# croci/bluest

Hardware: AMD Instinct MI355X
Metric: Phi-assemblies/s (higher is better)
Workload: dtype f64; 1 GPU; n=20 models, groups up to size 5 (K_tot=21699), n_out=8, Wishart covariances; one step = V and grad V of one allocation for all outputs; n_models=20, k_max=5, K_tot=21699, n_out=8, batch=1, parallelism=single GPU, evaluation=stored group inverses, launch=hipGraph replay of 20-step graphs (20 of 20 steps), rest eager

## Files before the change

bluest_amd/csrc/plan.hip:

```cpp

#include "common.hpp"

static int g_debug_timing = getenv("BLUEST_DEBUG_TIMING") ? 1 : 0;
struct PhaseTimer {
    std::chrono::steady_clock::time_point t0 = std::chrono::steady_clock::now();
    const char *what;
    explicit PhaseTimer(const char *w) : what(w) {}
    void lap(const char *phase)
    {
        if (!g_debug_timing) return;
        const auto t1 = std::chrono::steady_clock::now();
        fprintf(stderr, "[bluest timing] %s: %s %.3f ms\n", what, phase, std::chrono::duration<double, std::milli>(t1 - t0).count());
        t0 = t1;
    }
};


#include "plan.hpp"
#include "spg_state.hpp"

template <typename COLT> __device__ __forceinline__ int4 load_cols4(const COLT *p);
template <> __device__ __forceinline__ int4 load_cols4<int32_t>(const int32_t *p) { return *reinterpret_cast<const int4 *>(p); }
template <> __device__ __forceinline__ int4 load_cols4<uint16_t>(const uint16_t *p)
{
// ... 139 lines not shown
                                                           double *__restrict__ v, int32_t *__restrict__ status,
                                                           const int32_t *__restrict__ gate, double *__restrict__ spg_state, int last_slot, int32_t *__restrict__ spg_enable,
                                                           unsigned int *__restrict__ ticket)
{
    __shared__ SolveLds<NT> lds;
    __shared__ double spg_ls[SPG_STATE_DOUBLES];
    __shared__ int s_closed;
    kernarg_now(N, n_out, rows, nsym, reg.Cd, reg.Co, reg.rank_ab, partial, n_chunks, gate, spg_state);
    const int o = blockIdx.x, c = blockIdx.y, tid = threadIdx.x;
    if (gate_closed(gate, &s_closed)) {
        if (spg_state && tid < WAVE && spg_closed_last(ticket + 16, gridDim.x * gridDim.y, tid))
            spg_decide_wave(spg_state, var, status, n_out, last_slot, spg_enable, spg_ls, tid);
        return;
    }
    SpgPrefetch pf;
    if (spg_state && tid < WAVE) spg_prefetch_state(spg_state, tid, pf);
    if (N < NT) { clear_pads(lds, N, tid, fold_threads(NT)); __syncthreads(); }
    fold_rows(lds, N, rows, o, nsym, partial + (int64_t)c * n_chunks, tid, fold_threads(NT), reg);
    __syncthreads();
    if (tid >= WAVE) return;
    const int lane = tid;
    if (spg_state) spg_prefetch_parts(pf, lane);
    const int64_t e = (int64_t)c * n_out + o;
    if (want_v & 2) {
        if (lane == 0) { var[e] = lds.at(0, 0); status[e] = 0; }
        return;
    }
    const double am = (lane < N) ? lds.amax[lane] : 0.0;
    const bool big = __ballot(am >= 0.05) != 0ull;
    const int reps = (want_v & 4) ? 2 : 1;
    double V_mine = 0.0;
    int32_t st_mine = 0;
    for (int rep = 0; rep < reps; rep++)
        solve_wave<NT>(lds, N, delta, am > 1.0e-6, am > 0.0, big, (want_v & 1) != 0, &V_mine, v + e * N, &st_mine, lane);
    if (lane == 0) { var[e] = V_mine; status[e] = st_mine; }
    if (spg_state) {
        int last = 0;
        if (n_out == 1) {
            spg_decide_wave(spg_state, var, status, n_out, last_slot, spg_enable, spg_ls, lane, pf, true, V_mine, st_mine);
            return;
        }
        if (lane == 0) {
            asm volatile("s_waitcnt vmcnt(0)" ::: "memory");
            __builtin_amdgcn_fence(__ATOMIC_RELEASE, "agent");
            asm volatile("s_waitcnt vmcnt(0)" ::: "memory");
            const unsigned int t = __hip_atomic_fetch_add(ticket, 1u, __ATOMIC_RELAXED, __HIP_MEMORY_SCOPE_AGENT);
            last = (t == (unsigned int)(n_out - 1)) ? 1 : 0;
            if (last) __hip_atomic_store(ticket, 0u, __ATOMIC_RELAXED, __HIP_MEMORY_SCOPE_AGENT);
        }
        last = __builtin_amdgcn_readfirstlane(last);
        if (last) {
            __builtin_amdgcn_fence(__ATOMIC_ACQUIRE, "agent");
            spg_decide_wave(spg_state, var, status, n_out, last_slot, spg_enable, spg_ls, lane, pf);
        }
    }
}

template <int NT>
__global__ __launch_bounds__(fold_threads(NT)) void k_fold_to_record(int N, int n_out, const RowDesc *__restrict__ rows, int nsym, FoldReg reg,
                                                        const double2 *__restrict__ partial, int64_t n_chunks,
                                                        double *__restrict__ rec)
{
    __shared__ SolveLds<NT> lds;
    kernarg_now(N, n_out, rows, nsym, reg.Cd, reg.Co, reg.rank_ab, partial, n_chunks, rec);
    const int o = blockIdx.x, c = blockIdx.y, tid = threadIdx.x;
    fold_rows(lds, N, rows, o, nsym, partial + (int64_t)c * n_chunks, tid, fold_threads(NT), reg);
    __syncthreads();
    const int reclen = N * N + 2 * N + 1;
    double *r = rec + ((int64_t)c * n_out + o) * reclen;
    for (int t = tid; t < N * N; t += fold_threads(NT)) r[t] = lds.at(t / N, t % N);
    if (tid >= WAVE) return;
    const double am = (tid < N) ? lds.amax[tid] : 0.0;
    if (tid < N) { r[N * N + tid] = (am > 1.0e-6) ? 1.0 : 0.0; r[N * N + N + tid] = (am > 0.0) ? 1.0 : 0.0; }
    const double big = wave_max(am);
    if (tid == 0) r[N * N + 2 * N] = (big >= 0.05) ? 1.0 : 0.0;
}

template <int NT>
__global__ __launch_bounds__(64) void k_solve_from_record(int N, int n_out, const double *__restrict__ rec,
                                                          double delta, int want_v, double *__restrict__ var,
                                                          double *__restrict__ v, int32_t *__restrict__ status)
{
    __shared__ SolveLds<NT> lds;
    const int o = blockIdx.x, c = blockIdx.y, lane = threadIdx.x;
    const int reclen = N * N + 2 * N + 1;
    const double *r = rec + ((int64_t)c * n_out + o) * reclen;
    clear_pads(lds, N, lane, WAVE);
    __syncthreads();
    for (int t = lane; t < N * N; t += WAVE) lds.at(t / N, t % N) = r[t];
    __syncthreads();
    const bool s1 = lane < N && r[N * N + lane] > 0.0;
    const bool s2 = lane < N && r[N * N + N + lane] > 0.0;
    const bool big = r[N * N + 2 * N] > 0.0;
    const int64_t e = (int64_t)c * n_out + o;
    solve_wave<NT>(lds, N, delta, s1, s2, big, (want_v & 1) != 0, var + e, v + e * N, status + e, lane);
}

__device__ __forceinline__ void jacobi_pinv_lds(double *A, double *Q, int N, int LD, int lane)
{
    for (int sweep = 0; sweep < 60; sweep++) {
        int rotated = 0;
        for (int p = 0; p < N - 1; p++)
            for (int q = p + 1; q < N; q++) {
                const double apq = A[p * LD + q], app = A[p * LD + p], aqq = A[q * LD + q];
                if (!(fabs(apq) > 1.0e-18 * sqrt(fabs(app * aqq)))) continue;
                rotated = 1;
                const double theta = (aqq - app) / (2.0 * apq);
                const double t = (theta >= 0 ? 1.0 : -1.0) / (fabs(theta) + sqrt(theta * theta + 1.0));
                const double c = 1.0 / sqrt(t * t + 1.0), sn = t * c;
                if (lane < N) {
                    const double arp = A[lane * LD + p], arq = A[lane * LD + q];
                    A[lane * LD + p] = c * arp - sn * arq;
                    A[lane * LD + q] = sn * arp + c * arq;
                    const double vrp = Q[lane * LD + p], vrq = Q[lane * LD + q];
                    Q[lane * LD + p] = c * vrp - sn * vrq;
                    Q[lane * LD + q] = sn * vrp + c * vrq;
                }
                wave_lds_sync();
                if (lane < N) {
                    const double apr = A[p * LD + lane], aqr = A[q * LD + lane];
                    A[p * LD + lane] = c * apr - sn * aqr;
                    A[q * LD + lane] = sn * apr + c * aqr;
                }
                wave_lds_sync();
            }
        if (!rotated) break;
    }
}
// ... 55 lines not shown
            }
            wave_lds_sync();
        }
    }
    if (lane < N) v[e * N + lane] = vmine;
    if (lane == 0) { var[e] = V; status[e] = st; }
}

template <int KU>
__global__ __launch_bounds__(256) void k_grad_tiles(const TileDesc *__restrict__ tiles, int64_t n_tiles,
                                                    const double *__restrict__ tvals, const double *__restrict__ v,
                                                    const int32_t *__restrict__ status, int N, int n_out, int n_cand,
                                                    double *__restrict__ grad, int64_t grad_stride,
                                                    const int32_t *__restrict__ gate)
{
    if (gate && *gate == 0) return;
    const int64_t t = (int64_t)blockIdx.x * 4 + (threadIdx.x >> 6);
    const int lane = threadIdx.x & 63;
    if (t >= n_tiles) return;
    const TileDesc td = tiles[t];
#define GT(KK) case KK: if (KK <= KU) { grad_tile<(KK <= KU ? KK : 1)>(td, tvals, v, status, N, n_out, n_cand, grad, grad_stride, lane); break; }
    switch (td.k) {
        GT(1) GT(2) GT(3) GT(4) GT(5) GT(6) GT(7) GT(8) GT(9) GT(10) GT(11) GT(12)
        default: grad_tile_generic(td, tvals, v, status, N, n_out, n_cand, grad, grad_stride, lane);
    }
#undef GT
}

__host__ __device__ constexpr int fused_tpb(int NT, int KU) { return (NT <= 26 && KU <= 8) ? 15 : 7; }
using SolveGradKuSet = InstSet<5, 6, 8, 12>;
using GradTilesKuSet = InstSet<5, 8, 12>;
using PhiObSet = InstSet<2, 4, 8>;
template <class F> static void solve_grad_ku_dispatch(int kmax, F &&launch) { SolveGradKuSet::dispatch(kmax, launch); }
constexpr uint32_t SG_HAS_REC = 1u, SG_HAS_GATE = 2u, SG_HAS_SPG = 4u;
template <int NT, int KU>
__global__ __launch_bounds__(64 * (fused_tpb(NT, KU) + 1)) void k_solve_grad(const double2 *__restrict__ partial, const uint16_t *__restrict__ rank_ab,
                                                    const RowDesc *__restrict__ rows, const TileDesc *__restrict__ tiles,
                                                    uint32_t n_nsym, int Cd, int Co, int bpo, uint32_t flags,
                                                    int n_out_arg, int tpb_arg, int tile_nt, const double *__restrict__ rec_arg, double delta,
                                                    const double *__restrict__ tvals,
                                                    double *__restrict__ var, double *__restrict__ v_ws,
                                                    int32_t *__restrict__ status, double *__restrict__ grad,
                                                    const int32_t *__restrict__ gate, double *__restrict__ spg_state_arg, int last_slot,
                                                    int32_t *__restrict__ spg_enable, unsigned int *__restrict__ ticket, const MaTail ma)
{
    constexpr int FUSED_TPB = fused_tpb(NT, KU);
    constexpr int NTHREADS = 64 * (FUSED_TPB + 1);
    constexpr int PU = tile_pairs(KU);
    __shared__ SolveLds<NT> lds;
    __shared__ double spg_ls[SPG_STATE_DOUBLES];
    const int N = (int)(n_nsym & 0xffu), nsym = (int)(n_nsym >> 8);
    const FoldReg reg{Cd, Co, rank_ab};
    const int tid = threadIdx.x, lane = tid & 63;
    const int wave = __builtin_amdgcn_readfirstlane(tid >> 6);
    int o, first, wg;
    if (bpo > 0) { o = blockIdx.y; first = blockIdx.x == 0; wg = o * bpo + blockIdx.x; }
    else { wg = blockIdx.x; const TileDesc td0 = tile_desc_uniform(tiles, (int64_t)wg * tpb_arg); o = td0.out; first = (td0.n_valid >> 30) & 1; }
    __shared__ int s_closed;
    double *spg_state = nullptr;
    if (flags & (SG_HAS_GATE | SG_HAS_SPG)) {
        if (flags & SG_HAS_SPG) spg_state = spg_state_arg;
        if ((flags & SG_HAS_GATE) && gate_closed(gate, &s_closed)) {
            if (spg_state && first && wave == 0 && spg_closed_last(ticket + 16, (unsigned int)n_out_arg, lane))
                spg_decide_wave(spg_state, var, status, n_out_arg, last_slot, spg_enable, spg_ls, lane);
            return;
        }
    }
    SpgPrefetch pf;
    if (spg_state && first && wave == 0) spg_prefetch_state(spg_state, lane, pf);
    if (N < NT) { clear_pads(lds, N, tid, NTHREADS); __syncthreads(); }
    const double *rec_o = (flags & SG_HAS_REC) ? rec_arg + (int64_t)o * (N * N + 2 * N + 1) : nullptr;
    if (rec_o) {
        for (int t = tid; t < N * N; t += NTHREADS) lds.at(t / N, t % N) = rec_o[t];
    } else {
        fold_rows<NT>(lds, N, rows, o, nsym, partial, tid, NTHREADS, reg,
                      [&]() { kernarg_now(n_out_arg, tpb_arg, delta, var, v_ws, status); });
    }
    const int n_out = uniform_value_here(n_out_arg), tpb = uniform_value_here(tpb_arg);
    const int64_t t0 = (int64_t)wg * tpb;
    TileDesc td;
    td.k = 1; td.n_valid = 0; td.val_off = td.grad_off = 0; td.out = (int16_t)o;
    if (wave > 0 && wave <= tpb) td = tile_desc_uniform(tiles, t0 + wave - 1);
    __syncthreads();
    const int k = td.k;
    double2 pr[PU];
    double V_pub = 0.0;
    int32_t st_pub = 0;
    if (wave == 0) {
        if (spg_state && first) spg_prefetch_parts(pf, lane);
        bool s1, s2, big;
        if (rec_o) {
            s1 = lane < N && rec_o[N * N + lane] > 0.0;
            s2 = lane < N && rec_o[N * N + N + lane] > 0.0;
            big = rec_o[N * N + 2 * N] > 0.0;
        } else {
            const double am = (lane < N) ? lds.amax[lane] : 0.0;
            s1 = am > 1.0e-6;
            s2 = am > 0.0;
            big = __ballot(am >= 0.05) != 0ull;
        }
        double V = 0.0;
        int32_t st = 0;
        solve_wave<NT>(lds, N, delta, s1, s2, big, true, &V, lds.vout, &st, lane);
        if (lane == 0) { lds.status = st; if (ma.x) lds.scratch[0] = V; }
        V_pub = V; st_pub = st;
        if (first) {
            if (lane == 0) { var[o] = V; status[o] = st; }
            if (lane < N) v_ws[(int64_t)o * N + lane] = lds.vout[lane];
        }
    } else if (k <= KU) {
        if (tile_nt) tile_load<PU, true>(pr, tvals + td.val_off, lane, tile_pairs(k));
        else tile_load(pr, tvals + td.val_off, lane, tile_pairs(k));
    }
    __syncthreads();
    if (wave == 0) {
        if (spg_state && first) {
            int last = 0;
            if (n_out == 1) {
                spg_decide_wave(spg_state, var, status, n_out, last_slot, spg_enable, spg_ls, lane, pf, true, V_pub, st_pub);
                return;
            }
            if (lane == 0) {
                asm volatile("s_waitcnt vmcnt(0)" ::: "memory");
                __builtin_amdgcn_fence(__ATOMIC_RELEASE, "agent");
                asm volatile("s_waitcnt vmcnt(0)" ::: "memory");
                const unsigned int t = __hip_atomic_fetch_add(ticket, 1u, __ATOMIC_RELAXED, __HIP_MEMORY_SCOPE_AGENT);
                last = (t == (unsigned int)(n_out - 1)) ? 1 : 0;
                if (last) __hip_atomic_store(ticket, 0u, __ATOMIC_RELAXED, __HIP_MEMORY_SCOPE_AGENT);
            }
            last = __builtin_amdgcn_readfirstlane(last);
            if (last) {
                __builtin_amdgcn_fence(__ATOMIC_ACQUIRE, "agent");
                spg_decide_wave(spg_state, var, status, n_out, last_slot, spg_enable, spg_ls, lane, pf);
            }
        }
        return;
    }
    const bool valid = lane < (td.n_valid & 0xffff);
    const bool inf = lds.status == BLUEST_EVAL_INF;
    double *gout = grad + td.grad_off + lane;
    const bool MA_ON = ma.x != nullptr;
#define GT(KK) case KK: if (KK <= KU) { const double q = tile_form<(KK <= KU ? KK : 1)>(pr, lds.vout);                                          \
        if (valid && !MA_ON) *gout = inf ? INFINITY : -q;                                                                                        \
        else if (valid && lds.status == BLUEST_EVAL_OK) { const int64_t i = td.grad_off + lane; const double so = ma.s[0], cci = ma.cc[i];       \
            const double xn = ma.x[i] * cci * ((1.0 / so) * q) / (lds.scratch[0] / so); ma.x[i] = xn; ma.m[i] = cci * xn; } break; }
    switch (k) {
        GT(1) GT(2) GT(3) GT(4) GT(5) GT(6) GT(7) GT(8) GT(9) GT(10) GT(11) GT(12)
        default: {
            const double *vl = lds.vout - (int64_t)td.out * N;
            const int32_t *sl = &lds.status - td.out;
            grad_tile_generic(td, tvals, vl, sl, N, n_out, 1, grad, 0, lane);
        }
    }
#undef GT
}

__global__ void k_combine_grad(const double *__restrict__ grad, int64_t grad_stride, const int64_t *__restrict__ goff,
                               const int32_t *__restrict__ invmap, int64_t L, int n_out,
                               const double *__restrict__ coef, const double *__restrict__ scale, int n_cand,
                               double *__restrict__ out, int64_t out_stride, const int32_t *__restrict__ gate)
{
    if (gate && *gate == 0) return;
    const int64_t j = (int64_t)blockIdx.x * blockDim.x + threadIdx.x;
    const int c = blockIdx.y;
    if (j >= L || c >= n_cand) return;
    double s = 0.0;
    for (int o = 0; o < n_out; o++) {
        const int32_t li = invmap[(int64_t)o * L + j];
        if (li >= 0) s = fma(coef[(int64_t)c * n_out + o], grad[(int64_t)c * grad_stride + goff[o] + li], s);
    }
    out[(int64_t)c * out_stride + j] = scale ? scale[j] * s : s;
}

// ... 690 lines not shown
extern "C" int bluest_plan_finalize(bluest_plan_t plan, int max_candidates)
{
    if (!plan) return fail(BLUEST_ERR_ARG, "plan is NULL");
    if (plan->finalized) return fail(BLUEST_ERR_STATE, "plan already finalized");
    if (plan->outs.empty()) return fail(BLUEST_ERR_STATE, "plan has no outputs");
    if (max_candidates <= 0 || max_candidates > 65535) return fail(BLUEST_ERR_ARG, "max_candidates=%d out of range", max_candidates);
    const int N = plan->N, n_out = (int)plan->outs.size();
    PhaseTimer timer("plan_finalize");

    plan->nsym = N * (N + 1) / 2;
    if (N > 64 || plan->nsym > 2080) return fail(BLUEST_ERR_ARG, "N=%d: the fused kernel's argument word holds N <= 64, nsym <= 2080", N);
    plan->max_cand = max_candidates;
    plan->shared = true;
    for (int o = 1; o < n_out; o++) {
        const OutputDesc &x = plan->outs[0], &y = plan->outs[o];
        if (x.K != y.K || x.sizes != y.sizes || x.groups != y.groups || x.mapping != y.mapping) { plan->shared = false; break; }
    }
    PlanLayout lay(n_out, plan->nsym, plan->shared ? 1 : n_out);
    int rc;
    if ((rc = layout_tiles(plan, lay))) return rc;
    plan->identity = plan->shared && plan->outs[0].L_o == plan->L;
    for (int64_t li = 0; plan->identity && li < plan->L; li++) plan->identity = plan->outs[0].mapping[li] == li;
    if ((rc = layout_phi(plan, lay, timer))) return rc;
    layout_fold_reg(plan, lay);
    timer.lap("CSR slots + columns");
    layout_invmap(plan, lay);
    plan->cols16 = plan->L <= 65536 && getenv("BLUEST_COLS32") == nullptr;
    plan->phi_ob_forced = 0;
    if (const char *e = getenv("BLUEST_PHI_OB")) { const int v = atoi(e); if (v == 2 || v == 4 || v == 8) plan->phi_ob_forced = v; }
    plan->phi_bytes = plan->n_chunks * lay.CH * 8 + (plan->shared ? plan->n_chunks / n_out : plan->n_chunks) * lay.CH * (plan->cols16 ? 2 : 4) + plan->n_chunks * 16;
    plan->grad_bytes = (int64_t)lay.n_tvals * 8 + plan->grad_len * 8;
    const char *nt_env = getenv("BLUEST_TILE_NT");
    plan->tile_nt = nt_env ? atoi(nt_env) != 0 : true;
    timer.lap("tile descriptors + inverse maps");
    if ((rc = arena_upload(plan, lay))) return rc;
    timer.lap("device arena + small uploads");
    if ((rc = scatter_values(plan, lay))) return rc;
    plan->finalized = true;
    if ((rc = mf_finalize(plan))) return rc;

    timer.lap("device scatter of the values");
    return BLUEST_OK;
}

int plan_ready(bluest_plan_t plan, int n_cand)
{
    if (!plan) return fail(BLUEST_ERR_ARG, "plan is NULL");
    if (!plan->finalized) return fail(BLUEST_ERR_STATE, "plan not finalized");
    if (n_cand <= 0 || n_cand > plan->max_cand) return fail(BLUEST_ERR_ARG, "n_cand=%d outside 1..%d", n_cand, plan->max_cand);
    return BLUEST_OK;
}

extern "C" int bluest_plan_output_layout(bluest_plan_t plan, int output, int *K, int64_t *sizes, int64_t *mapping)
{
    if (!plan || !K) return fail(BLUEST_ERR_ARG, "null pointer");
    if (output < 0 || output >= (int)plan->outs.size()) return fail(BLUEST_ERR_ARG, "output %d out of range", output);
    const OutputDesc &od = plan->outs[output];
    *K = od.K;
    if (sizes) std::copy(od.sizes.begin(), od.sizes.end(), sizes);
    if (mapping) std::copy(od.mapping.begin(), od.mapping.end(), mapping);
    return BLUEST_OK;
}

extern "C" int bluest_plan_restrict(bluest_plan_t parent, const int64_t *keep, int64_t n_keep, int max_candidates, bluest_plan_t *restricted)
{
    if (!parent || !keep || !restricted) return fail(BLUEST_ERR_ARG, "null pointer");
// ... 91 lines not shown
    return BLUEST_OK;
}

extern "C" int bluest_plan_traffic(bluest_plan_t plan, int64_t *phi_bytes, int64_t *grad_bytes)
{
    if (!plan) return fail(BLUEST_ERR_ARG, "plan is NULL");
    if (!plan->finalized) return fail(BLUEST_ERR_STATE, "plan not finalized");
    if (phi_bytes) *phi_bytes = plan->phi_bytes;
    if (grad_bytes) *grad_bytes = plan->grad_bytes;
    return BLUEST_OK;
}

extern "C" int bluest_plan_phi_len(bluest_plan_t plan, int64_t *len)
{
    if (!plan || !len) return fail(BLUEST_ERR_ARG, "null pointer");
    *len = (int64_t)plan->outs.size() * (plan->N * plan->N + 2 * plan->N + 1);
    return BLUEST_OK;
}

static void launch_grad(bluest_plan_t plan, const double *v_dev, const int32_t *status_dev, int n_cand, double *grad_dev,
                        int64_t grad_stride, hipStream_t st)
{
    GradTilesKuSet::dispatch(plan->kmax, [&](auto ku) {
        hipLaunchKernelGGL((k_grad_tiles<decltype(ku)::value>), dim3((unsigned)((plan->n_tiles + 3) / 4)), dim3(256), 0, st, plan->d_tiles,
                           plan->n_tiles, plan->d_tvals, v_dev, status_dev, plan->N, (int)plan->outs.size(), n_cand, grad_dev, grad_stride, plan->gate);
    });
}

static void launch_solve_from_record(bluest_plan_t plan, const double *rec, int n_cand, double delta, int want_v, double *var_dev,
                                     double *v_dev, int32_t *status_dev, hipStream_t st)
{
    const int n_out = (int)plan->outs.size();
    nt_dispatch(plan->N, [&](auto nt) {
        hipLaunchKernelGGL((k_solve_from_record<decltype(nt)::value>), dim3(n_out, n_cand), dim3(64), 0, st, plan->N, n_out, rec, delta, want_v,
                           var_dev, v_dev, status_dev);
    });
}

static void launch_solve_grad(bluest_plan_t plan, const double *rec, double delta, double *var_dev, int32_t *status_dev, double *grad_dev,
                              double *dec_state, int dec_last, int32_t *dec_enable, MaTail ma, hipStream_t st)
{
    const int n_out = (int)plan->outs.size();
    const dim3 grid = plan->fused_bpo > 0 ? dim3((unsigned)plan->fused_bpo, (unsigned)n_out) : dim3((unsigned)(plan->n_tiles / plan->fused_tpb));
    const uint32_t flags = (rec ? SG_HAS_REC : 0u) | (plan->gate ? SG_HAS_GATE : 0u) | (dec_state ? SG_HAS_SPG : 0u);
    nt_dispatch(plan->N, [&](auto nt) { solve_grad_ku_dispatch(plan->kmax, [&](auto ku) {
        constexpr int NT = decltype(nt)::value, KU = decltype(ku)::value;
        hipLaunchKernelGGL((k_solve_grad<NT, KU>), grid, dim3(64 * (fused_tpb(NT, KU) + 1)), 0, st, plan->d_partial, plan->fold_reg.rank_ab, plan->d_rows,
                           plan->d_tiles, (uint32_t)plan->N | (uint32_t)plan->nsym << 8, plan->fold_reg.Cd, plan->fold_reg.Co, plan->fused_bpo, flags,
                           n_out, plan->fused_tpb, (int)plan->tile_nt, rec, delta, plan->d_tvals, var_dev, plan->d_v, status_dev, grad_dev,
                           plan->gate, dec_state, dec_last, dec_enable, plan->d_ticket, ma);
    }); });
}

static const int64_t PHI_MIN_WAVES = 2304;
static int phi_ob(const bluest_plan_s *p, int n_cand)
{
    (void)n_cand;
    const int n_out = (int)p->outs.size();
    if (!p->shared || n_out < 2) return 0;
    if (p->phi_ob_forced) return p->phi_ob_forced;
    const int64_t ncpo = p->n_chunks / n_out;
    for (int i = PhiObSet::count - 1; i > 0; i--) {
        const int ob = PhiObSet::values[i];
        if (ob <= n_out && ncpo * ((n_out + ob - 1) / ob) >= PHI_MIN_WAVES) return ob;
    }
    return PhiObSet::values[0];
}

static void launch_chunks(bluest_plan_t p, const double *m, int n_cand, int64_t m_stride, hipStream_t st)
{
    const int n_out = (int)p->outs.size();
    const uint32_t flags = p->gate ? PHI_HAS_GATE : 0u;
    if (const int ob = phi_ob(p, n_cand)) {
        const int64_t ncpo = p->n_chunks / n_out;
        PhiObSet::dispatch(ob, [&](auto obc) {
            constexpr int OB = decltype(obc)::value;
#define LCS2(COLT) hipLaunchKernelGGL((k_phi_chunks_shared<OB, 1, COLT>), dim3((unsigned)ncpo, (n_out + OB - 1) / OB), dim3(64), 0, st, \
// ... 112 lines not shown
{
    if (!state_dev || !enable_dev || !status_dev || !grad_dev) return fail(BLUEST_ERR_ARG, "null pointer");
    if (plan && (int)plan->outs.size() > SPG_MAX_OUT) return fail(BLUEST_ERR_ARG, "more than %d outputs", SPG_MAX_OUT);
    return plan_eval(plan, m_dev, 1, 0, delta, var_dev, grad_dev, plan ? plan->grad_len : 0, status_dev, stream, state_dev, last_slot, enable_dev);
}

static int plan_eval(bluest_plan_t plan, const double *m_dev, int n_cand, int64_t m_stride, double delta,
                     double *var_dev, double *grad_dev, int64_t grad_stride, int32_t *status_dev, void *stream,
                     double *dec_state, int dec_last, int32_t *dec_enable, MaTail ma)
{
    int rc = plan_ready(plan, n_cand); if (rc) return rc;
    if (!m_dev || !var_dev) return fail(BLUEST_ERR_ARG, "null pointer");
    if (n_cand > 1 && m_stride < plan->L) return fail(BLUEST_ERR_ARG, "m_stride < L_global");
    if (grad_dev && n_cand > 1 && grad_stride < plan->grad_len) return fail(BLUEST_ERR_ARG, "grad_stride < grad_len");
    hipStream_t st = (hipStream_t)stream;
    const int n_out = (int)plan->outs.size();
    int32_t *status = status_dev ? status_dev : plan->d_status;
    if (plan->matfree && n_cand == 1 && !dec_state && !plan->gate) {
        const double *rec = nullptr;
        if ((rc = mf_phi_record(plan, m_dev, nullptr, &rec, st))) return rc;
        if (grad_dev) return mf_solve_grad(plan, rec, delta, var_dev, status, grad_dev, st, ma);
        launch_solve_from_record(plan, rec, 1, delta, plan->always_v ? 1 : 0, var_dev, plan->d_v, status, st);
        HIP_TRY(hipGetLastError());
        return BLUEST_OK;
    }
    launch_chunks(plan, m_dev, n_cand, m_stride, st);
    if (plan->mf_gradient && grad_dev && n_cand == 1 && !dec_state && !plan->gate)
        return mf_solve_grad(plan, nullptr, delta, var_dev, status, grad_dev, st, ma);
    if (grad_dev && n_cand == 1) {
        launch_solve_grad(plan, nullptr, delta, var_dev, status, grad_dev, dec_state, dec_last, dec_enable, ma, st);
        HIP_TRY(hipGetLastError());
        return BLUEST_OK;
    }
    const int want = (grad_dev || plan->always_v) ? 1 : 0;
    nt_dispatch(plan->N, [&](auto nt) {
        hipLaunchKernelGGL((k_solve_from_chunks<decltype(nt)::value>), dim3(n_out, n_cand), dim3(fold_threads(nt)), 0, st, plan->N, n_out, plan->d_rows,
                           plan->nsym, plan->fold_reg, plan->d_partial, plan->partial_stride, delta, want, var_dev, plan->d_v, status, plan->gate,
                           dec_state, dec_last, dec_enable, plan->d_ticket);
    });
    if (grad_dev)
        launch_grad(plan, plan->d_v, status, n_cand, grad_dev, grad_stride, st);
    HIP_TRY(hipGetLastError());
    return BLUEST_OK;
}

extern "C" int bluest_plan_is_identity(bluest_plan_t plan, int *yes)
{
    if (!plan || !yes) return fail(BLUEST_ERR_ARG, "null pointer");
    if (!plan->finalized) return fail(BLUEST_ERR_STATE, "plan not finalized");
    *yes = plan->identity ? 1 : 0;
    return BLUEST_OK;
}

static int eval_ma_kmax(const bluest_plan_s *plan)
{
    if (plan->outs.size() != 1 || !plan->identity || plan->gate) return 0;
    return plan->matfree ? 8 : 12;
}

extern "C" int bluest_plan_eval_ma_kmax(bluest_plan_t plan, int *kmax)
{
    if (!plan || !kmax) return fail(BLUEST_ERR_ARG, "null pointer");
    if (!plan->finalized) return fail(BLUEST_ERR_STATE, "plan not finalized");
    *kmax = eval_ma_kmax(plan);
    return BLUEST_OK;
}

extern "C" int bluest_plan_kmax(bluest_plan_t plan, int *kmax)
{
    if (!plan || !kmax) return fail(BLUEST_ERR_ARG, "null pointer");
    if (!plan->finalized) return fail(BLUEST_ERR_STATE, "plan not finalized");
    *kmax = plan->kmax;
    return BLUEST_OK;
}

extern "C" int bluest_plan_launch_config(bluest_plan_t plan, int n_cand, int32_t *cfg)
{
    if (!plan || !cfg) return fail(BLUEST_ERR_ARG, "null pointer");
    if (!plan->finalized) return fail(BLUEST_ERR_STATE, "plan not finalized");
    if (n_cand <= 0 || n_cand > plan->max_cand) return fail(BLUEST_ERR_ARG, "n_cand=%d outside 1..%d", n_cand, plan->max_cand);
    std::fill(cfg, cfg + BLUEST_LC_COUNT, 0);
    const bool one = n_cand == 1 && !plan->gate;
    cfg[BLUEST_LC_PATH] = (one && plan->matfree) ? 2 : (one && plan->mf_gradient) ? 3 : (n_cand == 1) ? 1 : 0;
    cfg[BLUEST_LC_PHI_OB] = phi_ob(plan, n_cand);
    cfg[BLUEST_LC_COLS16] = plan->cols16 ? 1 : 0;
    nt_dispatch(plan->N, [&](auto nt) {
        cfg[BLUEST_LC_NT] = decltype(nt)::value;
        cfg[BLUEST_LC_FOLD_THREADS] = fold_threads(decltype(nt)::value);
        solve_grad_ku_dispatch(plan->kmax, [&](auto ku) {
            cfg[BLUEST_LC_SOLVE_GRAD_KU] = decltype(ku)::value;
            cfg[BLUEST_LC_FUSED_TPB] = fused_tpb(decltype(nt)::value, decltype(ku)::value);
        });
    });
    cfg[BLUEST_LC_TILES_PER_WG] = plan->fused_tpb;
    GradTilesKuSet::dispatch(plan->kmax, [&](auto ku) { cfg[BLUEST_LC_GRAD_TILES_KU] = decltype(ku)::value; });
    cfg[BLUEST_LC_MATFREE] = plan->matfree ? 1 : (plan->mf_gradient ? 2 : 0);
    if (plan->mf_gradient) mf_instantiation(plan, &cfg[BLUEST_LC_MF_NW], &cfg[BLUEST_LC_MF_NT], &cfg[BLUEST_LC_MF_KU]);
    cfg[BLUEST_LC_ITERS] = plan->iters;
    cfg[BLUEST_LC_KMAX] = plan->kmax;
    return BLUEST_OK;
}

extern "C" int bluest_launch_set(int axis, int32_t *values, int cap, int *n)
{
    if (!n || (cap > 0 && !values)) return fail(BLUEST_ERR_ARG, "null pointer");
    std::vector<int32_t> s;
    auto add = [&](int v) { if (std::find(s.begin(), s.end(), v) == s.end()) s.push_back(v); };
    switch (axis) {
    case BLUEST_LC_PHI_OB: for (int v : PhiObSet::values) add(v); break;
    case BLUEST_LC_NT: for (int v : NtSet::values) add(v); break;
    case BLUEST_LC_FOLD_THREADS: for (int v : NtSet::values) add(fold_threads(v)); break;
    case BLUEST_LC_SOLVE_GRAD_KU: for (int v : SolveGradKuSet::values) add(v); break;
    case BLUEST_LC_FUSED_TPB: for (int nt : NtSet::values) for (int ku : SolveGradKuSet::values) add(fused_tpb(nt, ku)); break;
    case BLUEST_LC_GRAD_TILES_KU: for (int v : GradTilesKuSet::values) add(v); break;
    case BLUEST_LC_MF_NW: case BLUEST_LC_MF_NT: case BLUEST_LC_MF_KU: mf_instantiation_set(axis, s); break;
    default: return fail(BLUEST_ERR_ARG, "axis %d has no instantiation set", axis);
    }
    *n = (int)s.size();
    for (int i = 0; i < (int)s.size() && i < cap; i++) values[i] = s[(size_t)i];
    return BLUEST_OK;
}

extern "C" int bluest_plan_eval_ma(bluest_plan_t plan, double *m_dev, double *var_dev, int32_t *status_dev, const double *s_dev,
                                   const double *cc_dev, double *x_dev, void *stream)
{
    if (!plan || !m_dev || !var_dev || !status_dev || !s_dev || !cc_dev || !x_dev) return fail(BLUEST_ERR_ARG, "null pointer");
    if (!plan->finalized) return fail(BLUEST_ERR_STATE, "plan not finalized");
    if (plan->outs.size() != 1 || !plan->identity || plan->gate || plan->kmax > eval_ma_kmax(plan))
        return fail(BLUEST_ERR_STATE, "bluest_plan_eval_ma: one output on all groups under the identity mapping only, groups of at most %d models",
                    eval_ma_kmax(plan));
    return plan_eval(plan, m_dev, 1, 0, 0.0, var_dev, plan->d_v, plan->grad_len, status_dev, stream, nullptr, 0, nullptr, MaTail{x_dev, cc_dev, m_dev, s_dev});
}
// ... 14 lines not shown
```

bluest_amd/csrc/plan.hpp:

```cpp
#pragma once
#include "solve.hpp"

struct TileDesc {
    int64_t val_off;
    int64_t grad_off;
    int32_t n_valid;
    int16_t k, out;
};
__host__ __device__ constexpr int tile_ne(int k) { return k * (k + 1) / 2; }
__host__ __device__ constexpr int tile_ni(int k) { return (k + 7) / 8; }
__host__ __device__ constexpr int tile_slots(int k) { return (tile_ne(k) + tile_ni(k) + 1) & ~1; }
__host__ __device__ constexpr int tile_pairs(int k) { return tile_slots(k) / 2; }
__host__ __device__ constexpr int64_t tile_slot_off(int sl, int lane) { return (int64_t)(sl >> 1) * 128 + lane * 2 + (sl & 1); }

__device__ __forceinline__ TileDesc tile_desc_uniform(const TileDesc *__restrict__ tiles, int64_t t)
{
    static_assert(sizeof(TileDesc) == 24, "three 64-bit words");
    const auto *w = (const __attribute__((address_space(4))) uint64_t *)(tiles + t);
    const uint64_t w0 = w[0], w1 = w[1], w2 = w[2];
    TileDesc td;
    td.val_off = (int64_t)w0; td.grad_off = (int64_t)w1; td.n_valid = (int32_t)(uint32_t)w2;
    td.k = (int16_t)(uint16_t)(w2 >> 32); td.out = (int16_t)(uint16_t)(w2 >> 48);
    return td;
}


struct OutputDesc {
    int K = 0;
    std::vector<int64_t> sizes;
    std::vector<int64_t> groups;
    std::vector<int64_t> mapping;
    int64_t L_o = 0;
    int64_t n_inv = 0;
    double *d_invcov = nullptr;
    uint8_t *d_groups = nullptr;
    bool owns_groups = false;
    std::vector<double> h_C;
};

struct bluest_plan_s {
    int device = -1;
    int N = 0;
    int64_t L = 0;
    std::vector<OutputDesc> outs;
    bool finalized = false;
    int max_cand = 0;
    int iters = 1;
    bool shared = false;
    bool identity = false;
    int kmax = 0;
    bool spg_small = false;
    int fused_bpo = 0;
    int fused_tpb = 15;
    bool tile_nt = true;
    const int32_t *gate = nullptr;
    bool always_v = false;
    int nsym = 0;
    int64_t n_chunks = 0, n_tiles = 0, grad_len = 0;
    std::vector<int64_t> grad_off;
    int64_t phi_bytes = 0, grad_bytes = 0;
    double *d_vals = nullptr;
    int32_t *d_cols = nullptr;
    bool cols16 = false;
    int phi_ob_forced = 0;
    RowDesc *d_rows = nullptr;
    TileDesc *d_tiles = nullptr;
    double *d_tvals = nullptr;
    int32_t *d_invmap = nullptr;
    int64_t *d_goff = nullptr;
    FoldReg fold_reg = {0, 0, nullptr};
    int32_t *d_pslot = nullptr;
    int64_t partial_stride = 0;
    int slots_per_output = 0;
    double2 *d_partial = nullptr;
    double *d_v = nullptr;
    void *d_arena = nullptr;
    void *d_scratch = nullptr;
    size_t scratch_bytes = 0;
    int32_t *d_status = nullptr;
    unsigned int *d_ticket = nullptr;
    bool matfree = false;
    bool mf_gradient = false;
    void *mf = nullptr;
    void *d_master = nullptr;
    size_t master_bytes = 0;
    std::vector<std::vector<int32_t>> inv_host;
};

struct DeviceScope {
    int prev = -1;
    bool switched = false;
    explicit DeviceScope(int dev)
    {
        if (hipGetDevice(&prev) == hipSuccess && prev != dev && dev >= 0) switched = hipSetDevice(dev) == hipSuccess;
    }
    ~DeviceScope() { if (switched) (void)hipSetDevice(prev); }
};


typedef double tile_d2v __attribute__((ext_vector_type(2)));
template <int PU, bool NT = false>
__device__ __forceinline__ void tile_load(double2 (&pr)[PU], const double *__restrict__ tile, int lane, int n_pairs)
{
    const char *base = reinterpret_cast<const char *>(tile);
    const uint32_t lo = 16u * (uint32_t)lane;
#pragma unroll
    for (int i = 0; i < PU; i++)
        if (i < n_pairs) {
            const char *p = (base + (lo + 4096u * (i >> 2))) + 1024 * (i & 3);
            if (NT) { const tile_d2v v = __builtin_nontemporal_load(reinterpret_cast<const tile_d2v *>(p)); pr[i] = make_double2(v.x, v.y); }
            else pr[i] = *reinterpret_cast<const double2 *>(p);
        }
}
template <int PU>
__device__ __forceinline__ double tile_slot(const double2 (&pr)[PU], int sl) { return (sl & 1) ? pr[sl >> 1].y : pr[sl >> 1].x; }

template <int K, int PU>
__device__ __forceinline__ double tile_form(const double2 (&pr)[PU], const double *__restrict__ vc)
{
    constexpr int NI = tile_ni(K);
    double vj[K];
#pragma unroll
    for (int j = 0; j < K; j++) {
        const double sl = tile_slot(pr, j >> 3);
        const unsigned w = (unsigned)((j & 4) ? __double2hiint(sl) : __double2loint(sl));
        vj[j] = vc[(w >> (8 * (j & 3))) & 0xffu];
    }
    double q = 0.0;
    int e = NI;
#pragma unroll
    for (int j = 0; j < K; j++) {
        double t = 0.0;
#pragma unroll
        for (int l = j + 1; l < K; l++) t = fma(tile_slot(pr, e + (l - j)), vj[l], t);
        t = fma(tile_slot(pr, e), vj[j], 2.0 * t);
        q = fma(vj[j], t, q);
        e += K - j;
    }
    return q;
}

template <int K>
__device__ __forceinline__ void grad_tile(const TileDesc &td, const double *__restrict__ tvals, const double *__restrict__ v,
                                          const int32_t *__restrict__ status, int N, int n_out, int n_cand,
                                          double *__restrict__ grad, int64_t grad_stride, int lane)
{
// ... 51 lines not shown
```

bluest_amd/csrc/solve.hpp:

```cpp
#pragma once
#include "common.hpp"

struct RowDesc {
    int32_t first_chunk;
    int32_t n_chunks;
    int16_t out, a, b, pad;
};


template <int NT>
struct SolveLds {
    static constexpr int LDP = NT + 2;
    double phi[NT * LDP];
    double amax[NT];
    double vout[NT];
    double scratch[NT <= 32 && NT > 16 ? 16 * (NT - 15) : 1];
    int status;
    __device__ __forceinline__ double &at(int a, int b) { return phi[(NT - 1 - a) * LDP + (NT - 1 - b)]; }
};

template <int NT>
__device__ __forceinline__ void clear_pads(SolveLds<NT> &lds, int N, int tid, int nthreads)
{
    if (N < NT)
// ... 243 lines not shown
        return (lane == NT - 1) ? rl : -a[NT - 1] * rinv_mine * rl;
    } else {
        constexpr int E = M::E;
        asm volatile("s_nop 4" ::: "memory");
        GjExtraStep<NT, 0>::run(a, lane, rinv_mine);
        GjDppStep<NT, E>::run(a, lane, rinv_mine, last_pivot);
        last_pivot = readlane_f64(last_pivot, 0);
        const bool ok = rinv_mine > 0.0 && rinv_mine * (BLUEST_PIVOT_TOL * diag0) < 1.0;
        bad |= (__ballot(!ok && lane < M::n_lanes) != 0ull || !isfinite(last_pivot)) ? 1 : 0;
        const double rl = readlane_f64(rinv_mine, M::lane_of(NT - 1));
        double x = (lane == M::lane_of(NT - 1)) ? rl : -a[NT - 1] * rinv_mine * rl;
        if constexpr (E > 0) {
            if (lane < 16) {
#pragma unroll
                for (int e = 0; e < E; e++) scratch[lane * (E + 1) + e] = a[e];
                scratch[lane * (E + 1) + E] = x;
            }
            wave_lds_sync();
            const int e_mine = (lane >= 16 && lane < 16 + E) ? lane - 16 : 0;
            double acc = 0.0;
#pragma unroll
            for (int l = 0; l < 16; l++) acc = fma(scratch[l * (E + 1) + e_mine], scratch[l * (E + 1) + E], acc);
            wave_lds_sync();
            double xe = 0.0;
            asm volatile("s_nop 4" ::: "memory");
            GjBackSub<NT, E>::run(a, lane, rinv_mine, acc, xe);
            x = (lane >= 16) ? xe : x;
        }
        return x;
    }
}

template <int NT>
__device__ __forceinline__ void solve_wave(SolveLds<NT> &lds, int N, double delta, bool s1, bool s2, bool big_in, bool want_v,
                                        double *__restrict__ var_out, double *__restrict__ v_out,
                                        int32_t *__restrict__ status_out, int lane)
{
    constexpr int LDP = SolveLds<NT>::LDP;
    const unsigned long long mask1 = __ballot(lane < N && s1);
    const unsigned long long mask2 = (delta != 0.0) ? __ballot(lane < N) : __ballot(lane < N && s2);
    const unsigned long long all = (N >= 64) ? ~0ull : ((1ull << N) - 1ull);
    const bool big = uniform_i(big_in ? 1 : 0) != 0;
    int status = BLUEST_EVAL_OK;
    double V = 0.0;
    double vmine = 0.0;
    unsigned long long vmask = 0ull;
    int vswap = 0;
    const int p = GjMap<NT>::pos_of(lane);
    if (__builtin_expect(!big, 0)) {
        status = BLUEST_EVAL_INF;
        V = INFINITY;
    } else if (__builtin_expect(mask1 == 0ull, 0)) {
        status = BLUEST_EVAL_NO_MODEL0;
        V = NAN;
    } else {
        if (__builtin_expect(!(mask1 & 1ull), 0)) status = BLUEST_EVAL_NO_MODEL0;
        const int npass = (mask1 == mask2 || !want_v) ? 1 : 2;
        for (int pass = 0; pass < npass; pass++) {
            unsigned long long mask = (pass == 0) ? mask1 : mask2;
            if (__builtin_expect(pass == 1 && !(mask & 1ull), 0)) break;
            const int t = __ffsll((long long)mask) - 1;
            int mp = NT - 1 - p;
            if (__builtin_expect(t != 0, 0)) {
                mp = (mp == 0) ? t : (mp == t ? 0 : mp);
                mask = (mask | 1ull) & ~(1ull << t);
            }
            const bool mine = (NT - 1 - p) < N && ((mask >> (NT - 1 - p)) & 1ull);
            const double *row = lds.phi + (NT - 1 - mp) * LDP;
            double a[NT];
// ... 73 lines not shown
```

bluest_amd/plan.py:

```python
import ctypes

import numpy as np
import torch

from . import _lib
from ._lib import check, ptr

EVAL_OK, EVAL_INF, EVAL_NO_MODEL0, EVAL_SINGULAR = 0, 1, 2, 3

LAUNCH_FIELDS = ("path", "phi_ob", "cols16", "nt", "fold_threads", "solve_grad_ku", "fused_tpb", "tiles_per_wg", "grad_tiles_ku",
                 "matfree", "mf_nw", "mf_nt", "mf_ku", "iters", "kmax")
LAUNCH_AXES = ("phi_ob", "nt", "fold_threads", "solve_grad_ku", "fused_tpb", "grad_tiles_ku", "mf_nw", "mf_nt", "mf_ku")


def launch_sets():
    L = _lib.lib()
    out = {}
    for axis in LAUNCH_AXES:
        n = ctypes.c_int(0)
        check(L.bluest_launch_set(LAUNCH_FIELDS.index(axis), None, 0, ctypes.byref(n)))
        vals = np.zeros(n.value, dtype=np.int32)
        check(L.bluest_launch_set(LAUNCH_FIELDS.index(axis), ptr(vals), n.value, ctypes.byref(n)))
        out[axis] = [int(v) for v in vals]
    return out


def _stream():
    return ctypes.c_void_p(torch.cuda.current_stream().cuda_stream)


def _i64(a):
    return np.ascontiguousarray(a, dtype=np.int64)


def _f64(a):
    return np.ascontiguousarray(a, dtype=np.float64)


def require_cuda():
    if not torch.cuda.is_available():
        raise _lib.BluestHipError("no GPU visible to torch: bluest_amd computes on MI355X only (no CPU fallback)")


class _LazyInverses(object):
# ... 269 lines not shown
```

include/bluest_hip.h:

```cpp
#ifndef BLUEST_HIP_H
#define BLUEST_HIP_H

#include <stdint.h>

#ifdef __cplusplus
extern "C" {
#endif

#define BLUEST_ABI_VERSION 1

#define BLUEST_OK          0
#define BLUEST_ERR_ARG     1
#define BLUEST_ERR_HIP     2
#define BLUEST_ERR_NOGPU   3
#define BLUEST_ERR_STATE   4

#define BLUEST_MAX_MODELS  64
#define BLUEST_MAX_GROUP   32

#define BLUEST_EVAL_OK         0
#define BLUEST_EVAL_INF        1
#define BLUEST_EVAL_NO_MODEL0  2
#define BLUEST_EVAL_SINGULAR   3

// ... 120 lines not shown
int bluest_xchg_status(bluest_xchg_t xchg, int64_t *calls, int *timed_out);
int bluest_xchg_destroy(bluest_xchg_t xchg);

int bluest_master_max_support(bluest_plan_t plan, int *s_max);
int bluest_master_newton(bluest_plan_t plan, int S, const int64_t *support_host, const double *cc_host, const double *s_dev,
                         const double *bg_dev, double eps_bg, double *x_dev, double *mu_dev, double tol, int maxit,
                         double *out_dev, void *stream);
int bluest_master_newton_capped(bluest_plan_t plan, int S, const int64_t *support_host, const double *cc_host, const double *s_dev,
                                const double *bg_dev, double eps_bg, double *x_dev, double *mu_dev, double tol, int maxit,
                                double *out_dev, int ncap, const int32_t *cap_model_host, const double *cap_b_host, double *nu_dev,
                                void *stream);
int bluest_ma_update(bluest_plan_t plan, const double *var_dev, const int32_t *status_dev, const double *grad_dev,
                     const double *s_dev, const double *cc_dev, double p, double *x_dev, double *m_dev, void *stream);
int bluest_plan_is_identity(bluest_plan_t plan, int *yes);
int bluest_plan_eval_ma(bluest_plan_t plan, double *m_dev, double *var_dev, int32_t *status_dev, const double *s_dev,
                        const double *cc_dev, double *x_dev, void *stream);
int bluest_plan_eval_ma_kmax(bluest_plan_t plan, int *kmax);
int bluest_plan_kmax(bluest_plan_t plan, int *kmax);
#define BLUEST_LC_PATH           0
#define BLUEST_LC_PHI_OB         1
#define BLUEST_LC_COLS16         2
#define BLUEST_LC_NT             3
#define BLUEST_LC_FOLD_THREADS   4
#define BLUEST_LC_SOLVE_GRAD_KU  5
#define BLUEST_LC_FUSED_TPB      6
#define BLUEST_LC_TILES_PER_WG   7
#define BLUEST_LC_GRAD_TILES_KU  8
#define BLUEST_LC_MATFREE        9
#define BLUEST_LC_MF_NW         10
#define BLUEST_LC_MF_NT         11
#define BLUEST_LC_MF_KU         12
#define BLUEST_LC_ITERS         13
#define BLUEST_LC_KMAX          14
#define BLUEST_LC_COUNT         15
int bluest_plan_launch_config(bluest_plan_t plan, int n_cand, int32_t *cfg);
int bluest_launch_set(int axis, int32_t *values, int cap, int *n);
int bluest_wave_reduce_probe(const double *in_dev, int64_t n_rows, double *sum_dev, double *max_dev, double *quad_dev,
                             int64_t *isum_dev, void *stream);
int bluest_wave_reduce_multi_probe(const double *in_dev, int64_t n_rows, int ob, double *out_dev, void *stream);
int bluest_support_point(int64_t L, int S, const int64_t *sup_dev, const double *xs_dev, const double *cc_dev, double eps,
                         double *m_dev, void *stream);
#define BLUEST_PRICE_CANDIDATES 1024
int bluest_price(bluest_plan_t plan, const double *grad_dev, const double *mu_dev, const double *s_dev, const double *cc_dev,
                 int S, const int64_t *sup_dev, double *c_sup_dev, double *top_val_dev, int64_t *top_idx_dev, double *y0_dev,
                 void *stream);

int bluest_price_capped(bluest_plan_t plan, const double *grad_dev, const double *mu_dev, const double *s_dev, const double *cc_dev,
                        int S, const int64_t *sup_dev, double *c_sup_dev, double *top_val_dev, int64_t *top_idx_dev, double *y0_dev,
                        const uint64_t *capmask_dev, const double *nu_dev, const double *master_out_dev, void *stream);

#define BLUEST_MFMC_MAX_NEIGHBOURS 30
#define BLUEST_MFMC_MAX_ROUND      24
#define BLUEST_MFMC_MAX_OUTPUTS    64
#define BLUEST_MFMC_BUDGET         1
#define BLUEST_MFMC_CONTINUOUS     2
#define BLUEST_MFMC_SMALL_BUDGET   4
#define BLUEST_MFMC_OK             0
#define BLUEST_MFMC_NONE           1
#define BLUEST_MFMC_TOO_BIG        2
int bluest_mfmc_search(int nb, int n_out, int flags, double budget, const double *eps2, const double *epsm2, const double *w,
                       const double *s, const double *rho, const int32_t *perm, const uint32_t *adj, uint32_t *best_mask,
                       uint32_t *best_combo, double *best_obj, int32_t *status, void *stream);

#define BLUEST_COVPROJ_OK          0
#define BLUEST_COVPROJ_MAXIT       1
#define BLUEST_COVPROJ_MAXFEV      2
#define BLUEST_COVPROJ_NONFINITE   3
// ... 51 lines not shown
```

Before: 814,000 assemblies/s (one output: Phi(m) over all groups -> V, grad V).

## Add fast all-active Gauss-Jordan solve path and hoist tile address setup

Adds a fast path in the wave solver: when every model is active and well-scaled (checked with ballots), it runs a register-resident Gauss-Jordan elimination for the last column instead of the general masked solve. The general path can be forced with an env var and a flag bit. The fused solve-grad kernel also computes tile base pointers and lane offsets before the barrier, uses global address-space vector loads, and passes more kernel arguments to the early kernarg prefetch. This is meant to cut solve latency and address arithmetic on the critical path, at the cost of extra register pressure and a second solver whose accuracy differs on near-singular inputs.

```diff
diff --git a/bluest_amd/csrc/plan.hip b/bluest_amd/csrc/plan.hip
--- a/bluest_amd/csrc/plan.hip
+++ b/bluest_amd/csrc/plan.hip
@@ -195,7 +195,7 @@
     double V_mine = 0.0;
     int32_t st_mine = 0;
     for (int rep = 0; rep < reps; rep++)
-        solve_wave<NT>(lds, N, delta, am > 1.0e-6, am > 0.0, big, (want_v & 1) != 0, &V_mine, v + e * N, &st_mine, lane);
+        solve_wave<NT>(lds, N, delta, am > 1.0e-6, am > 0.0, big, (want_v & 1) != 0, &V_mine, v + e * N, &st_mine, lane, (want_v & 8) != 0);
     if (lane == 0) { var[e] = V_mine; status[e] = st_mine; }
     if (spg_state) {
         int last = 0;
@@ -256,7 +256,7 @@
     const bool s2 = lane < N && r[N * N + N + lane] > 0.0;
     const bool big = r[N * N + 2 * N] > 0.0;
     const int64_t e = (int64_t)c * n_out + o;
-    solve_wave<NT>(lds, N, delta, s1, s2, big, (want_v & 1) != 0, var + e, v + e * N, status + e, lane);
+    solve_wave<NT>(lds, N, delta, s1, s2, big, (want_v & 1) != 0, var + e, v + e * N, status + e, lane, (want_v & 8) != 0);
 }
 
 __device__ __forceinline__ void jacobi_pinv_lds(double *A, double *Q, int N, int LD, int lane)
@@ -378,7 +378,7 @@
 using GradTilesKuSet = InstSet<5, 8, 12>;
 using PhiObSet = InstSet<2, 4, 8>;
 template <class F> static void solve_grad_ku_dispatch(int kmax, F &&launch) { SolveGradKuSet::dispatch(kmax, launch); }
-constexpr uint32_t SG_HAS_REC = 1u, SG_HAS_GATE = 2u, SG_HAS_SPG = 4u;
+constexpr uint32_t SG_HAS_REC = 1u, SG_HAS_GATE = 2u, SG_HAS_SPG = 4u, SG_GENERAL = 8u;
 template <int NT, int KU>
 __global__ __launch_bounds__(64 * (fused_tpb(NT, KU) + 1)) void k_solve_grad(const double2 *__restrict__ partial, const uint16_t *__restrict__ rank_ab,
                                                     const RowDesc *__restrict__ rows, const TileDesc *__restrict__ tiles,
@@ -420,15 +420,25 @@
         for (int t = tid; t < N * N; t += NTHREADS) lds.at(t / N, t % N) = rec_o[t];
     } else {
         fold_rows<NT>(lds, N, rows, o, nsym, partial, tid, NTHREADS, reg,
-                      [&]() { kernarg_now(n_out_arg, tpb_arg, delta, var, v_ws, status); });
+                      [&]() { kernarg_now(n_out_arg, tpb_arg, delta, tvals, var, v_ws, status, grad, ma.x, ma.cc, ma.m, ma.s); });
     }
     const int n_out = uniform_value_here(n_out_arg), tpb = uniform_value_here(tpb_arg);
     const int64_t t0 = (int64_t)wg * tpb;
     TileDesc td;
     td.k = 1; td.n_valid = 0; td.val_off = td.grad_off = 0; td.out = (int16_t)o;
     if (wave > 0 && wave <= tpb) td = tile_desc_uniform(tiles, t0 + wave - 1);
+    const int k = td.k;
+    tile_gptr tile_base = nullptr;
+    double *gbase = nullptr;
+    int n_pairs = 0;
+    uint32_t lane_off = 0;
+    if (wave > 0) {
+        tile_base = uniform_value_here(tile_global(tvals + td.val_off));
+        gbase = uniform_value_here(grad + td.grad_off);
+        n_pairs = uniform_value_here(k <= KU ? tile_pairs(k) : 0);
+        lane_off = lane_value_here(16u * (uint32_t)lane);
+    }
     __syncthreads();
-    const int k = td.k;
     double2 pr[PU];
     double V_pub = 0.0;
     int32_t st_pub = 0;
@@ -447,7 +457,7 @@
         }
         double V = 0.0;
         int32_t st = 0;
-        solve_wave<NT>(lds, N, delta, s1, s2, big, true, &V, lds.vout, &st, lane);
+        solve_wave<NT>(lds, N, delta, s1, s2, big, true, &V, lds.vout, &st, lane, (flags & SG_GENERAL) != 0);
         if (lane == 0) { lds.status = st; if (ma.x) lds.scratch[0] = V; }
         V_pub = V; st_pub = st;
         if (first) {
@@ -455,8 +465,8 @@
             if (lane < N) v_ws[(int64_t)o * N + lane] = lds.vout[lane];
         }
     } else if (k <= KU) {
-        if (tile_nt) tile_load<PU, true>(pr, tvals + td.val_off, lane, tile_pairs(k));
-        else tile_load(pr, tvals + td.val_off, lane, tile_pairs(k));
+        if (tile_nt) tile_load_at<PU, true>(pr, tile_base, lane_off, n_pairs);
+        else tile_load_at<PU, false>(pr, tile_base, lane_off, n_pairs);
     }
     __syncthreads();
     if (wave == 0) {
@@ -484,7 +494,7 @@
     }
     const bool valid = lane < (td.n_valid & 0xffff);
     const bool inf = lds.status == BLUEST_EVAL_INF;
-    double *gout = grad + td.grad_off + lane;
+    double *gout = gbase + lane;
     const bool MA_ON = ma.x != nullptr;
 #define GT(KK) case KK: if (KK <= KU) { const double q = tile_form<(KK <= KU ? KK : 1)>(pr, lds.vout);                                          \
         if (valid && !MA_ON) *gout = inf ? INFINITY : -q;                                                                                        \
@@ -1241,6 +1251,8 @@
     plan->grad_bytes = (int64_t)lay.n_tvals * 8 + plan->grad_len * 8;
     const char *nt_env = getenv("BLUEST_TILE_NT");
     plan->tile_nt = nt_env ? atoi(nt_env) != 0 : true;
+    const char *sg_env = getenv("BLUEST_SOLVE_GENERAL");
+    plan->solve_general = sg_env && atoi(sg_env) != 0;
     timer.lap("tile descriptors + inverse maps");
     if ((rc = arena_upload(plan, lay))) return rc;
     timer.lap("device arena + small uploads");
@@ -1398,7 +1410,8 @@
 {
     const int n_out = (int)plan->outs.size();
     nt_dispatch(plan->N, [&](auto nt) {
-        hipLaunchKernelGGL((k_solve_from_record<decltype(nt)::value>), dim3(n_out, n_cand), dim3(64), 0, st, plan->N, n_out, rec, delta, want_v,
+        hipLaunchKernelGGL((k_solve_from_record<decltype(nt)::value>), dim3(n_out, n_cand), dim3(64), 0, st, plan->N, n_out, rec, delta,
+                           want_v | (plan->solve_general ? 8 : 0),
                            var_dev, v_dev, status_dev);
     });
 }
@@ -1408,7 +1421,8 @@
 {
     const int n_out = (int)plan->outs.size();
     const dim3 grid = plan->fused_bpo > 0 ? dim3((unsigned)plan->fused_bpo, (unsigned)n_out) : dim3((unsigned)(plan->n_tiles / plan->fused_tpb));
-    const uint32_t flags = (rec ? SG_HAS_REC : 0u) | (plan->gate ? SG_HAS_GATE : 0u) | (dec_state ? SG_HAS_SPG : 0u);
+    const uint32_t flags = (rec ? SG_HAS_REC : 0u) | (plan->gate ? SG_HAS_GATE : 0u) | (dec_state ? SG_HAS_SPG : 0u) |
+                           (plan->solve_general ? SG_GENERAL : 0u);
     nt_dispatch(plan->N, [&](auto nt) { solve_grad_ku_dispatch(plan->kmax, [&](auto ku) {
         constexpr int NT = decltype(nt)::value, KU = decltype(ku)::value;
         hipLaunchKernelGGL((k_solve_grad<NT, KU>), grid, dim3(64 * (fused_tpb(NT, KU) + 1)), 0, st, plan->d_partial, plan->fold_reg.rank_ab, plan->d_rows,
@@ -1587,7 +1601,7 @@
         HIP_TRY(hipGetLastError());
         return BLUEST_OK;
     }
-    const int want = (grad_dev || plan->always_v) ? 1 : 0;
+    const int want = ((grad_dev || plan->always_v) ? 1 : 0) | (plan->solve_general ? 8 : 0);
     nt_dispatch(plan->N, [&](auto nt) {
         hipLaunchKernelGGL((k_solve_from_chunks<decltype(nt)::value>), dim3(n_out, n_cand), dim3(fold_threads(nt)), 0, st, plan->N, n_out, plan->d_rows,
                            plan->nsym, plan->fold_reg, plan->d_partial, plan->partial_stride, delta, want, var_dev, plan->d_v, status, plan->gate,
@@ -1653,6 +1667,7 @@
     if (plan->mf_gradient) mf_instantiation(plan, &cfg[BLUEST_LC_MF_NW], &cfg[BLUEST_LC_MF_NT], &cfg[BLUEST_LC_MF_KU]);
     cfg[BLUEST_LC_ITERS] = plan->iters;
     cfg[BLUEST_LC_KMAX] = plan->kmax;
+    cfg[BLUEST_LC_SOLVE_GENERAL] = plan->solve_general ? 1 : 0;
     return BLUEST_OK;
 }
 
diff --git a/bluest_amd/csrc/plan.hpp b/bluest_amd/csrc/plan.hpp
--- a/bluest_amd/csrc/plan.hpp
+++ b/bluest_amd/csrc/plan.hpp
@@ -53,6 +53,7 @@
     int fused_bpo = 0;
     int fused_tpb = 15;
     bool tile_nt = true;
+    bool solve_general = false;
     const int32_t *gate = nullptr;
     bool always_v = false;
     int nsym = 0;
@@ -112,6 +113,20 @@
             else pr[i] = *reinterpret_cast<const double2 *>(p);
         }
 }
+typedef const __attribute__((address_space(1))) char *tile_gptr;
+__device__ __forceinline__ tile_gptr tile_global(const double *tile) { return (tile_gptr)reinterpret_cast<const char *>(tile); }
+template <int PU, bool NT>
+__device__ __forceinline__ void tile_load_at(double2 (&pr)[PU], tile_gptr base, uint32_t lo, int n_pairs)
+{
+    typedef const __attribute__((address_space(1))) tile_d2v *vptr;
+#pragma unroll
+    for (int i = 0; i < PU; i++)
+        if (i < n_pairs) {
+            const vptr p = (vptr)((base + (lo + 4096u * (i >> 2))) + 1024 * (i & 3));
+            const tile_d2v v = NT ? __builtin_nontemporal_load(p) : *p;
+            pr[i] = make_double2(v.x, v.y);
+        }
+}
 template <int PU>
 __device__ __forceinline__ double tile_slot(const double2 (&pr)[PU], int sl) { return (sl & 1) ? pr[sl >> 1].y : pr[sl >> 1].x; }
 
diff --git a/bluest_amd/csrc/solve.hpp b/bluest_amd/csrc/solve.hpp
--- a/bluest_amd/csrc/solve.hpp
+++ b/bluest_amd/csrc/solve.hpp
@@ -299,9 +299,61 @@
 }
 
 template <int NT>
+__device__ __forceinline__ void solve_wave_all(SolveLds<NT> &lds, int N, double delta, bool want_v, double *__restrict__ var_out,
+                                               double *__restrict__ v_out, int32_t *__restrict__ status_out, int lane)
+{
+    constexpr int LDP = SolveLds<NT>::LDP;
+    const int p = GjMap<NT>::pos_of(lane);
+    const double *row = lds.phi + p * LDP;
+    double a[NT];
+#pragma unroll
+    for (int c = 0; c < NT; c += 2) {
+        const double2 x = *reinterpret_cast<const double2 *>(row + c);
+        a[c] = x.x; a[c + 1] = x.y;
+    }
+    const bool mine = (NT - 1 - p) < N;
+    const double diag0 = row[p] + (mine ? delta : 1.0);
+#pragma unroll
+    for (int c = 0; c < NT; c++) a[c] = (c == p) ? diag0 : a[c];
+    double last_pivot = 1.0;
+    int bad = 0;
+    const double x = gj_solve_last<NT>(a, lane, diag0, lds.scratch, last_pivot, bad);
+    const bool sing = uniform_i(bad) != 0;
+    if (want_v) {
+        if (lane < GjMap<NT>::n_lanes && mine) v_out[NT - 1 - p] = sing ? NAN : x;
+        wave_lds_sync();
+    }
+    if (lane == 0) { *var_out = sing ? NAN : 1.0 / last_pivot; *status_out = sing ? BLUEST_EVAL_SINGULAR : BLUEST_EVAL_OK; }
+}
+
+template <int NT>
+__device__ __forceinline__ void solve_wave_general(SolveLds<NT> &lds, int N, double delta, bool s1, bool s2, bool big_in, bool want_v,
+                                                   double *__restrict__ var_out, double *__restrict__ v_out,
+                                                   int32_t *__restrict__ status_out, int lane);
+
+template <int NT>
 __device__ __forceinline__ void solve_wave(SolveLds<NT> &lds, int N, double delta, bool s1, bool s2, bool big_in, bool want_v,
-                                        double *__restrict__ var_out, double *__restrict__ v_out,
-                                        int32_t *__restrict__ status_out, int lane)
+                                           double *__restrict__ var_out, double *__restrict__ v_out,
+                                           int32_t *__restrict__ status_out, int lane, bool general = false)
+{
+    if constexpr (GjMap<NT>::dpp) {
+        const unsigned long long in1 = __ballot(lane < N && s1 && big_in);
+        const unsigned long long in2 = __ballot(lane < N && (s2 || delta != 0.0));
+        const unsigned long long all = (1ull << N) - 1ull;
+        if (__builtin_expect((in1 & in2) == all && !general, 1)) {
+            solve_wave_all<NT>(lds, N, delta, want_v, var_out, v_out, status_out, lane);
+            return;
+        }
+        N = uniform_value_here(N);
+        lane = lane_value_here(lane);
+    }
+    solve_wave_general<NT>(lds, N, delta, s1, s2, big_in, want_v, var_out, v_out, status_out, lane);
+}
+
+template <int NT>
+__device__ __forceinline__ void solve_wave_general(SolveLds<NT> &lds, int N, double delta, bool s1, bool s2, bool big_in, bool want_v,
+                                                   double *__restrict__ var_out, double *__restrict__ v_out,
+                                                   int32_t *__restrict__ status_out, int lane)
 {
     constexpr int LDP = SolveLds<NT>::LDP;
     const unsigned long long mask1 = __ballot(lane < N && s1);
diff --git a/bluest_amd/plan.py b/bluest_amd/plan.py
--- a/bluest_amd/plan.py
+++ b/bluest_amd/plan.py
@@ -9,7 +9,7 @@
 EVAL_OK, EVAL_INF, EVAL_NO_MODEL0, EVAL_SINGULAR = 0, 1, 2, 3
 
 LAUNCH_FIELDS = ("path", "phi_ob", "cols16", "nt", "fold_threads", "solve_grad_ku", "fused_tpb", "tiles_per_wg", "grad_tiles_ku",
-                 "matfree", "mf_nw", "mf_nt", "mf_ku", "iters", "kmax")
+                 "matfree", "mf_nw", "mf_nt", "mf_ku", "iters", "kmax", "solve_general")
 LAUNCH_AXES = ("phi_ob", "nt", "fold_threads", "solve_grad_ku", "fused_tpb", "grad_tiles_ku", "mf_nw", "mf_nt", "mf_ku")
 
 
diff --git a/include/bluest_hip.h b/include/bluest_hip.h
--- a/include/bluest_hip.h
+++ b/include/bluest_hip.h
@@ -176,7 +176,8 @@
 #define BLUEST_LC_MF_KU         12
 #define BLUEST_LC_ITERS         13
 #define BLUEST_LC_KMAX          14
-#define BLUEST_LC_COUNT         15
+#define BLUEST_LC_SOLVE_GENERAL 15
+#define BLUEST_LC_COUNT         16
 int bluest_plan_launch_config(bluest_plan_t plan, int n_cand, int32_t *cfg);
 int bluest_launch_set(int axis, int32_t *values, int cap, int *n);
 int bluest_wave_reduce_probe(const double *in_dev, int64_t n_rows, double *sum_dev, double *max_dev, double *quad_dev,
```

Result: slower. 797,400 assemblies/s (one output: Phi(m) over all groups -> V, grad V) (-2.0%).
